# jhuldr/BrainFM

Hardware: AMD Instinct MI355X
Metric: voxels/sec whole-volume multi-task inference, 256^3 tiled (higher is better)
Workload: dtype f16x3-split (fp32-grade); 1 GPU; 256^3 volume, reference tiling win160/stride80 -> 27 tiles, UNet3D f64 x6 levels, 9 heads (69 ch), fused tail + deformed atlas + on-device stitch of 17 keys; stitched_keys=17, mfma_passes=3, submission=hipGraph replay per tile shape, parallelism=tiles sharded over 1 rank(s), gather to rank 0, tiles_in_flight_per_gpu=2

## Files before the change

### brainfm_amd/csrc/conv3d_wino4.hip

```cpp
#include "wino_shared.h"
#include <cstdlib>
#include <type_traits>

namespace {

typedef _Float16 half8 __attribute__((ext_vector_type(8)));
typedef float floatx16 __attribute__((ext_vector_type(16)));
typedef __fp16 fp16x2_t __attribute__((ext_vector_type(2)));

constexpr int KC = 16;
constexpr int NPOS = 6;
constexpr int NTHR = 256;
constexpr int NRG = NTHR / 32;
constexpr int MLD = 33;

struct W4Params {
    const float* A;
    int CA, D, H, W;
    const float *scale, *shift, *bound;
    int G;
    const uint4* wp;
    int wexp, Cout;
    float slope;
    float* out;
// ... 367 lines not shown
                float MN = INFINITY, MX = -INFINITY;
#pragma unroll
                for (int r = 0; r < NRG; ++r) {
                    Ssum += ls[r * 32 + tid]; Q += lq[r * 32 + tid];
                    MN = fminf(MN, lmn[r * 32 + tid]); MX = fmaxf(MX, lmx[r * 32 + tid]);
                }
                const size_t o = (size_t)mt * p.Cout + nt * 64 + nb * 32 + tid;
                p.rsum[o] = Ssum; p.rsq[o] = Q; p.rmn[o] = MN; p.rmx[o] = MX;
            }
        }
    }
}

template <int NPASS>
__global__ void __launch_bounds__(NTHR, 2) conv_wino4(const W4Params p) { conv_wino4_body<NPASS, 0>(p); }
template <int NPASS>
__global__ void __launch_bounds__(NTHR, 2) conv_wino4_masked(const W4Params p) { conv_wino4_body<NPASS, 1>(p); }

constexpr int DB_TD = 8, DB_TH = 8, DB_HT = 10, DB_NROW = 100;
constexpr int DB_PLANE = DB_NROW * 16;
constexpr int DB_RAWROW = 6 * 64;
constexpr int DB_RAW = DB_NROW * DB_RAWROW;
constexpr int DB_NDMA = DB_NROW / 2;
constexpr int DB_NDMA_WAVE = (DB_NDMA + 3) / 4;

template <bool LO>
__device__ __forceinline__ void split_store4_mix(const float (&t)[4], unsigned char* dp, int plane_stride) {
    const fp16x2_t h01 = __builtin_amdgcn_cvt_pkrtz(t[0], t[1]);
    const fp16x2_t h23 = __builtin_amdgcn_cvt_pkrtz(t[2], t[3]);
    uint2 hv;
    hv.x = __builtin_bit_cast(unsigned, h01);
    hv.y = __builtin_bit_cast(unsigned, h23);
    *reinterpret_cast<uint2*>(dp) = hv;
    if constexpr (LO) {
        uint2 lv;
        asm("v_fma_mixlo_f16 %0, %1, -1.0, %2 op_sel_hi:[1,0,0]" : "=v"(lv.x) : "v"(hv.x), "v"(t[0]));
        asm("v_fma_mixhi_f16 %0, %1, -1.0, %2 op_sel:[1,0,0] op_sel_hi:[1,0,0]" : "+v"(lv.x) : "v"(hv.x), "v"(t[1]));
        asm("v_fma_mixlo_f16 %0, %1, -1.0, %2 op_sel_hi:[1,0,0]" : "=v"(lv.y) : "v"(hv.y), "v"(t[2]));
        asm("v_fma_mixhi_f16 %0, %1, -1.0, %2 op_sel:[1,0,0] op_sel_hi:[1,0,0]" : "+v"(lv.y) : "v"(hv.y), "v"(t[3]));
        *reinterpret_cast<uint2*>(dp + plane_stride) = lv;
    }
}

template <int NPASS, int MODE, int ABL = 0>
__device__ __forceinline__ void conv_wino4d_body(const W4Params& pin) {
    W4Params p = pin;
    constexpr bool LIST = MODE != 0;
    constexpr bool UNI = MODE == 3;
    constexpr bool BY_FLAG = MODE == 2 || MODE == 3;
    constexpr int NPL = (NPASS == 3) ? 2 : 1;
    constexpr int NF = 2 * NPL;
    constexpr int NWF = 3 * NPL;
    constexpr int RAW_OFF = 2 * NPOS * NPL * DB_PLANE;
    extern __shared__ __attribute__((aligned(16))) unsigned char lds[];

    const int tid = threadIdx.x;
    const int lane = tid & 63;
    const int wv = __builtin_amdgcn_readfirstlane(tid >> 6);
    const int posA = wv;
    const int posB = 4 + (wv >> 1), nbB = wv & 1;
    const int l32 = lane & 31, khalf = lane >> 5;
#ifdef BFM_W4_ABLATE
    if (p.dbg_sleep > 0 && blockIdx.x < 512) {
        unsigned hwid;
        asm volatile("s_getreg_b32 %0, hwreg(HW_REG_HW_ID)" : "=s"(hwid));
        if (hwid & 1)
            for (int i = 0; i < p.dbg_sleep; ++i) __builtin_amdgcn_s_sleep(16);
    }
#endif
    int item;
    {
        const int nblk = LIST ? p.list_n[0] * p.NT : p.nMt * p.NT;
        const int bid = blockIdx.x;
        if (LIST && bid >= nblk) return;
        const int q = nblk >> 3, r = nblk & 7;
        const int xcd = bid & 7, idx = bid >> 3;
        item = (xcd < r ? xcd * (q + 1) : r * (q + 1) + (xcd - r) * q) + idx;
    }
    const int mt = LIST ? p.list[item / p.NT] : item / p.NT;
    const int nt = item % p.NT;
    int mtl = mt;
    if (!LIST && p.nMtS > 0) {
        const int smp = mt / p.nMtS;
        mtl = mt - smp * p.nMtS;
        p.A += smp * p.sA;
        p.out += smp * p.sO;
        p.scale += smp * p.saff;
        p.shift += smp * p.saff;
        p.bound += smp * p.G;
    }
    const int tx = mtl % p.nTx;
    const int ty = (mtl / p.nTx) % p.nTy;
    const int tz = mtl / (p.nTx * p.nTy);
    const int z0 = tz * DB_TD, y0 = ty * DB_TH, x0 = tx * 4;
    int cls = 0;
    if constexpr (BY_FLAG) cls = __builtin_amdgcn_readfirstlane((int)p.uni_flags[mt]);
    const bool rep = MODE == 2 && cls != 0;
    float4* const ybuf = BY_FLAG && cls ? reinterpret_cast<float4*>(p.uni_acc) + ((size_t)(cls - 1) * p.NT + nt) * (2 * 8 * NTHR) + tid
                                        : nullptr;

    float bmax = 0.f;
    for (int g = 0; g < p.G; ++g) bmax = fmaxf(bmax, p.bound[g]);
    int aexp = 0;
    if (bmax > 0.f && bmax < INFINITY) {
        int ex;
        (void)frexpf(bmax, &ex);
        aexp = 10 - ex;
        aexp = aexp > 60 ? 60 : (aexp < -60 ? -60 : aexp);
    }
    const float a_scale = ldexpf(1.0f, aexp);
    const float dq = ldexpf(1.0f, -(aexp + p.wexp));

    floatx16 acc[2][2];
    floatx16 accB[2];
    if constexpr (!UNI) {
    int a_off[4];
#pragma unroll
    for (int u = 0; u < 4; ++u) {
        const int pos = u < 2 ? posA : posB, mb = u & 1;
        const int pr = row_perm(l32);
        const int d = mb * 2 + (pr >> 4) + 4 * ((pr & 15) >> 3), h = pr & 7;
        a_off[u] = ((pos * 2 + khalf) * NPL) * DB_PLANE + (d * DB_HT + h) * 16;
    }

    const int q4 = tid & 3;
    int msk[2];
#pragma unroll
    for (int it = 0; it < 2; ++it) {
        const int r = (tid >> 2) + 64 * it;
        msk[it] = -1;
        if (r < DB_NROW) {
            const int hz = r / DB_HT, hy = r - hz * DB_HT;
            const int gz = z0 + hz - 1, gy = y0 + hy - 1;
            int m = 0;
            if (gz >= 0 && gz < p.D && gy >= 0 && gy < p.H) {
#pragma unroll
                for (int i = 0; i < 6; ++i)
                    if (x0 - 1 + i >= 0 && x0 - 1 + i < p.W) m |= 1 << i;
            }
            msk[it] = m;
        }
    }
    const bool inner = z0 >= 1 && z0 + DB_TD < p.D && y0 >= 1 && y0 + DB_TH < p.H && x0 >= 1 && x0 + 4 < p.W;
    const int st_plane = ((q4 >> 1) * NPL) * DB_PLANE + (q4 & 1) * 8;

    const int slot = lane >> 2;
    const int sb = slot >= 6 ? 1 : 0;
    int gxc = x0 + (slot - 6 * sb) - 1;
    gxc = gxc < 0 ? 0 : (gxc > p.W - 1 ? p.W - 1 : gxc);
    const int lane_el = gxc * p.CA + (lane & 3) * 4;
    const bool dma_lane = slot < 12;
    const unsigned raw_lds = (unsigned)(__UINTPTR_TYPE__)((__attribute__((address_space(3))) unsigned char*)(lds + RAW_OFF));
    const int zs = z0 > 0 ? z0 - 1 : 0;
    const float* slab = p.A + (int64_t)zs * p.H * p.W * p.CA;
    auto issue_dma = [&](int kc) __attribute__((always_inline)) {
        if constexpr ((ABL & 8) != 0) return;
        if (dma_lane) {
            int wvo = wv;
            asm volatile("" : "+s"(wvo));
#pragma unroll
            for (int n = 0; n < DB_NDMA_WAVE; ++n) {
                const int i = wvo + 4 * n;
                if (n < DB_NDMA_WAVE - 1 || i < DB_NDMA) {
                    const int hz = i / 5, hp = i - 5 * hz;
                    int gz = z0 + hz - 1;
                    gz = gz < 0 ? 0 : (gz > p.D - 1 ? p.D - 1 : gz);
                    int gy0 = y0 + 2 * hp - 1, gy1 = gy0 + 1;
                    gy0 = gy0 < 0 ? 0 : (gy0 > p.H - 1 ? p.H - 1 : gy0);
                    gy1 = gy1 > p.H - 1 ? p.H - 1 : gy1;
                    const unsigned ro0 = (unsigned)((((gz - zs) * p.H + gy0) * p.W) * p.CA);
                    const unsigned ro1 = (unsigned)((((gz - zs) * p.H + gy1) * p.W) * p.CA);
                    const unsigned vo = ((sb ? ro1 : ro0) + (unsigned)lane_el) * 4u;
                    const unsigned la = raw_lds + (unsigned)(i * (2 * DB_RAWROW));
                    asm volatile("s_mov_b32 m0, %2\n\ts_nop 0\n\tglobal_load_lds_dwordx4 %0, %1" ::"v"(vo), "s"(slab + kc * KC), "s"(la)
                                 : "memory");
                }
            }
        }
    };

#pragma unroll
    for (int u = 0; u < 2; ++u) {
#pragma unroll
        for (int i = 0; i < 16; ++i) { acc[u][0][i] = 0.f; acc[u][1][i] = 0.f; accB[u][i] = 0.f; }
    }

// ... 11 lines not shown
    };
    issue_dma(0);
    fetch(0, wq[0]);
    fetch(1, wq[1]);
    half8 a_abl[4][NPL];
    if constexpr ((ABL & 2) != 0) {
#pragma unroll
        for (int u = 0; u < 4; ++u)
#pragma unroll
            for (int hl = 0; hl < NPL; ++hl)
#pragma unroll
                for (int j = 0; j < 8; ++j) a_abl[u][hl][j] = (_Float16)(0.01f * (float)((lane * 7 + u * 3 + hl * 5 + j) % 61) - 0.3f);
    }

    for (int kc = 0; kc < p.KCN; ++kc) {
        const int c0 = kc * KC;
        const float4 sc4 = *reinterpret_cast<const float4*>(p.scale + c0 + q4 * 4);
        const float4 sh4 = *reinterpret_cast<const float4*>(p.shift + c0 + q4 * 4);
        const float sc[4] = {sc4.x * a_scale, sc4.y * a_scale, sc4.z * a_scale, sc4.w * a_scale};
        const float sh[4] = {sh4.x * a_scale, sh4.y * a_scale, sh4.z * a_scale, sh4.w * a_scale};
        __builtin_amdgcn_s_waitcnt(0x0F70);
        __syncthreads();
#pragma unroll
        for (int it = 0; it < 2; ++it) {
            if (msk[it] < 0) continue;
            if constexpr ((ABL & 4) != 0) continue;
            const int r = (tid >> 2) + 64 * it;
            const float4* rp = reinterpret_cast<const float4*>(
                __builtin_assume_aligned(lds + RAW_OFF + r * DB_RAWROW + q4 * 16, 16));
            float4 v[6];
#pragma unroll
            for (int i = 0; i < 6; ++i) v[i] = rp[i * 4];
            float dd[6][4];
            if (inner) {
#pragma unroll
                for (int i = 0; i < 6; ++i) {
                    const float y[4] = {v[i].x, v[i].y, v[i].z, v[i].w};
#pragma unroll
                    for (int c = 0; c < 4; ++c) dd[i][c] = fmaf(y[c], sc[c], sh[c]);
                }
            } else {
#pragma unroll
                for (int i = 0; i < 6; ++i) {
                    const bool ok = msk[it] & (1 << i);
                    const float y[4] = {v[i].x, v[i].y, v[i].z, v[i].w};
#pragma unroll
                    for (int c = 0; c < 4; ++c) {
                        const float a = fmaf(y[c], sc[c], sh[c]);
                        dd[i][c] = ok ? a : 0.f;
                    }
// ... 63 lines not shown
                    const half8 bhi = __builtin_bit_cast(half8, wq[cur][NF]);
                    if constexpr (NPASS == 3) {
                        const half8 blo = __builtin_bit_cast(half8, wq[cur][NF + 1]);
                        accB[u - 2] = __builtin_amdgcn_mfma_f32_32x32x16_f16(a[1], bhi, accB[u - 2], 0, 0, 0);
                        accB[u - 2] = __builtin_amdgcn_mfma_f32_32x32x16_f16(a[0], blo, accB[u - 2], 0, 0, 0);
                    }
                    accB[u - 2] = __builtin_amdgcn_mfma_f32_32x32x16_f16(a[0], bhi, accB[u - 2], 0, 0, 0);
                }
            }
        }
    }

    }

    if constexpr ((ABL & 16) != 0) {
        float sm = 0.f;
#pragma unroll
        for (int u = 0; u < 2; ++u)
#pragma unroll
            for (int i = 0; i < 16; ++i) sm += acc[u][0][i] + acc[u][1][i] + accB[u][i];
        if (sm == 12345.678f) p.out[tid] = sm;
        return;
    }
    float* m = reinterpret_cast<float*>(lds);
    const int col = tid & 31, rg = tid >> 5;
    const bool interior = z0 + DB_TD <= p.D && y0 + DB_TH <= p.H && x0 + 4 <= p.W;
    int un[4];
#pragma unroll
    for (int c = 0; c < 4; ++c) un[c] = row_unperm(16 * (c >> 1) + 8 * (c & 1) + rg);
    const unsigned off_t = (unsigned)((rg * p.W) * p.Cout + col);
#pragma unroll
    for (int nb = 0; nb < 2; ++nb) {
        if constexpr (!UNI && (ABL & 256) == 0) {
        __syncthreads();
#pragma unroll
        for (int u = 0; u < 2; ++u) {
            float* mw = m + (posA * 64 + u * 32 + khalf * 4) * MLD + l32;
#pragma unroll
            for (int i = 0; i < 16; ++i)
                mw[((i >> 2) * 8 + (i & 3)) * MLD] = acc[u][nb][i];
        }
        if (nbB == nb) {
#pragma unroll
            for (int u = 0; u < 2; ++u) {
                float* mw = m + (posB * 64 + u * 32 + khalf * 4) * MLD + l32;
#pragma unroll
                for (int i = 0; i < 16; ++i)
                    mw[((i >> 2) * 8 + (i & 3)) * MLD] = accB[u][i];
// ... 65 lines not shown
                    const float* mr = mc + qr * MLD;
                    const float m0 = mr[0 * 64 * MLD], m1 = mr[1 * 64 * MLD], m2 = mr[2 * 64 * MLD];
                    const float m3 = mr[3 * 64 * MLD], m4 = mr[4 * 64 * MLD], m5 = mr[5 * 64 * MLD];
                    const float s1 = m1 + m2, d1 = m1 - m2, s2 = m3 + m4, d2 = m3 - m4;
                    y[0] = ((m0 + s1) + s2) * dq;
                    y[1] = fmaf(2.f, d2, d1) * dq;
                    y[2] = fmaf(4.f, s2, s1) * dq;
                    y[3] = (fmaf(8.f, d2, d1) + m5) * dq;
                    if (MODE == 2 && rep) ybuf[(nb * 8 + it) * NTHR] = make_float4(y[0], y[1], y[2], y[3]);
                }
#pragma unroll
                for (int k = 0; k < 4; ++k) {
                    if (x0 + k < p.W) {
                        float r = y[k];
                        if (p.accum) r = r + o[off_t + (unsigned)(k * p.Cout)];
                        r = r >= 0.f ? r : r * p.slope;
                        o[off_t + (unsigned)(k * p.Cout)] = r;
                        fs += r; fq = fmaf(r, r, fq); fmn = fminf(fmn, r); fmx = fmaxf(fmx, r);
                    }
                }
            }
        }
        if (p.rsum != nullptr) {
            double* ls = reinterpret_cast<double*>(lds + (UNI ? (size_t)0 : (size_t)NPOS * 64 * MLD * sizeof(float)));
            double* lq = ls + NRG * 32;
            float* lmn = reinterpret_cast<float*>(lq + NRG * 32);
            float* lmx = lmn + NRG * 32;
            ls[rg * 32 + col] = (double)fs; lq[rg * 32 + col] = (double)fq;
            lmn[rg * 32 + col] = fmn; lmx[rg * 32 + col] = fmx;
            __syncthreads();
            if (tid < 32) {
                double Ssum = 0.0, Q = 0.0;
                float MN = INFINITY, MX = -INFINITY;
#pragma unroll
                for (int r = 0; r < NRG; ++r) {
                    Ssum += ls[r * 32 + tid]; Q += lq[r * 32 + tid];
                    MN = fminf(MN, lmn[r * 32 + tid]); MX = fmaxf(MX, lmx[r * 32 + tid]);
                }
                const size_t o = (size_t)mt * p.Cout + nt * 64 + nb * 32 + tid;
                p.rsum[o] = Ssum; p.rsq[o] = Q; p.rmn[o] = MN; p.rmx[o] = MX;
            }
        }
    }
}

template <int NPASS>
__global__ void __launch_bounds__(NTHR, 2) conv_wino4d(const W4Params p) { conv_wino4d_body<NPASS, 0>(p); }
template <int NPASS>
__global__ void __launch_bounds__(NTHR, 2) conv_wino4d_masked(const W4Params p) { conv_wino4d_body<NPASS, 1>(p); }
template <int NPASS>
__global__ void __launch_bounds__(NTHR, 2) conv_wino4d_rest(const W4Params p) { conv_wino4d_body<NPASS, 2>(p); }
template <int NPASS>
__global__ void __launch_bounds__(NTHR, 2) conv_wino4d_uniform(const W4Params p) { conv_wino4d_body<NPASS, 3>(p); }
#ifdef BFM_W4_ABLATE
template <int ABL>
__global__ void __launch_bounds__(NTHR, 2) conv_wino4d_abl(const W4Params p) { conv_wino4d_body<3, 0, ABL>(p); }
#endif

__global__ void pack_wino4(const float* __restrict__ w, int Cin, int Cout, int wexp, int npl, uint4* __restrict__ out) {
    const int KCN = Cin / KC;
    const int nf = 2 * npl;
    const int64_t n = (int64_t)(Cout / 64) * NPOS * KCN * 9 * nf * 64;
    const double s = ldexp(1.0, wexp);
    for (int64_t i = (int64_t)blockIdx.x * blockDim.x + threadIdx.x; i < n; i += (int64_t)gridDim.x * blockDim.x) {
        const int lane = (int)(i & 63);
        int64_t r = i >> 6;
        const int f = (int)(r % nf); r /= nf;
        const int t = (int)(r % 9); r /= 9;
        const int kc = (int)(r % KCN); r /= KCN;
        const int ps = (int)(r % NPOS); r /= NPOS;
        const int ntile = (int)r;
        const int nb = f / npl, hl = f - nb * npl;
        const int co = ntile * 64 + nb * 32 + (lane & 31);
        const int ci0 = kc * KC + 8 * (lane >> 5);
        half8 v;
#pragma unroll
// ... 12 lines not shown
        }
        out[i] = __builtin_bit_cast(uint4, v);
    }
}

int ilog2i(int v) { int r = 0; while ((1 << r) < v) ++r; return r; }

bool choose_box4(int D, int H, int W, int npl, int& TD, int& TH, int& TW) {
    if (!bfm_wino_choose_box(D, H, W, npl, TD, TH, TW)) return false;
    if (TW % 4 || TD * TH * (TW / 4) != 64) return false;
    const int64_t npos = (int64_t)(TD + 2) * (TH + 2) * (TW / 4);
    if (npos * 4 > 3 * NTHR) return false;
    const int64_t plane = ((npos * 16 + 255) / 256) * 256 + 16;
    return 2 * NPOS * npl * plane <= 62 * 1024;
}

bool use_dma_kernel(int D, int H, int W) {
#ifdef BFM_W4_ABLATE
    if (getenv("BFM_W4_OLD")) return false;
#endif
    return D >= DB_TD && H >= DB_TH && W >= 4;
}

bool choose_box_any(int D, int H, int W, int npl, int& TD, int& TH, int& TW) {
    if (use_dma_kernel(D, H, W)) { TD = DB_TD; TH = DB_TH; TW = 4; return true; }
    return choose_box4(D, H, W, npl, TD, TH, TW);
}

}

extern "C" size_t bfm_pack_conv_weights_wino4_bytes(int Cin, int Cout, int passes) {
    if (Cin <= 0 || Cout <= 0 || Cin % KC || Cout % 64) return 0;
    const int npl = passes == 3 ? 2 : 1;
    return (size_t)(Cout / 64) * NPOS * (Cin / KC) * 9 * 2 * npl * 64 * sizeof(uint4);
}

extern "C" int bfm_pack_conv_weights_wino4(const float* w_oidhw, int Cin, int Cout, float wmax_abs_host, int passes,
                                           void* wpacked, int* wexp_host, bfm_stream_t stream) {
    if (!w_oidhw || !wpacked || !wexp_host || Cin <= 0 || Cout <= 0) return BFM_E_ARG;
    if (Cin % KC || Cout % 64 || (passes != 1 && passes != 3)) return BFM_E_SHAPE;
    int wexp = 0;
    if (wmax_abs_host > 0.f && wmax_abs_host < INFINITY) {
        int ex;
        (void)frexpf(wmax_abs_host, &ex);
        wexp = 14 - ex;
        wexp = wexp > 60 ? 60 : (wexp < -60 ? -60 : wexp);
// ... 7 lines not shown
    return bfm_launch_status();
}

extern "C" int bfm_conv3x3x3_wino4_rows(int D, int H, int W, int passes) {
    int TD, TH, TW;
    if (D <= 0 || H <= 0 || W <= 0 || !choose_box_any(D, H, W, passes == 3 ? 2 : 1, TD, TH, TW)) return 0;
    return (int)bfm_box_count(D, H, W, TD, TH, TW);
}

extern "C" int bfm_conv3x3x3_wino4_box(int D, int H, int W, int passes, int* box) {
    int TD, TH, TW;
    if (!box || D <= 0 || H <= 0 || W <= 0 || !choose_box_any(D, H, W, passes == 3 ? 2 : 1, TD, TH, TW)) return BFM_E_ARG;
    box[0] = TD; box[1] = TH; box[2] = TW;
    return BFM_OK;
}

extern "C" size_t bfm_conv3x3x3_wino4_masked_workspace(int D, int H, int W, int passes) {
    const int n = bfm_conv3x3x3_wino4_rows(D, H, W, passes);
    if (n <= 0) return 0;
    return MaskListBuf::bytes((size_t)n);
}

static int w4_launch(const WinoLaunch& a) {
    if (const int rc = bfm_wino_check(a, KC)) return rc;
    const int D = a.D, H = a.H, W = a.W, CA = a.CA, Cout = a.Cout, passes = a.passes;
    const int S = a.batch.S, affine_stride = a.batch.affine_stride;
    const int npl = passes == 3 ? 2 : 1;
    W4Params p{};
    p.A = a.A; p.CA = CA; p.D = D; p.H = H; p.W = W;
    p.scale = a.scale; p.shift = a.shift; p.bound = a.bound; p.G = a.G;
    p.wp = static_cast<const uint4*>(a.wpacked);
    p.wexp = a.wexp; p.Cout = Cout; p.slope = a.slope; p.out = a.out; p.accum = a.flags & 1;
    if (!choose_box_any(D, H, W, npl, p.TD, p.TH, p.TW)) return BFM_E_SHAPE;
    const bool dma = use_dma_kernel(D, H, W);
    if (dma && (int64_t)(DB_TD + 2) * H * W * CA >= (int64_t)1 << 30) return BFM_E_SHAPE;
    p.HT = p.TH + 2; p.QW = p.TW / 4;
    p.qw_shift = ilog2i(p.QW); p.thq_shift = ilog2i(p.TH * p.QW);
    const int nTz = bfm_cdiv(D, p.TD);
    p.nTy = bfm_cdiv(H, p.TH); p.nTx = bfm_cdiv(W, p.TW);
    p.nMt = nTz * p.nTy * p.nTx;
    if (S > 1 || affine_stride > 0) {
        if (a.mask.img || S < 1 || (affine_stride != 0 && (affine_stride < CA || (affine_stride & 3)))) return BFM_E_ARG;
        p.nMtS = p.nMt;
        p.nMt = S * p.nMtS;
        p.saff = affine_stride > 0 ? affine_stride : CA;
        p.sA = (int64_t)D * H * W * CA;
        p.sO = (int64_t)D * H * W * Cout;
    }
    p.NT = Cout / 64;
    p.KCN = CA / KC;
    p.npos_lds = (p.TD + 2) * p.HT * p.QW;
    p.plane_stride = ((p.npos_lds * 16 + 255) / 256) * 256 + 16;
    size_t smem = dma ? (size_t)2 * NPOS * npl * DB_PLANE + DB_RAW : (size_t)2 * NPOS * npl * p.plane_stride;
    const size_t epi = (size_t)NPOS * 64 * MLD * sizeof(float) + (size_t)NRG * 32 * 24;
    if (smem < epi) smem = epi;
    if (smem > (dma ? 80u : 64u) * 1024) return BFM_E_SHAPE;
    const UniformFlagBuf fb{a.uniform.flags, (size_t)p.nMt};
    if (fb.flags) {
        int bd, bh, bw;
        if (!dma || a.mask.img || S > 1 || affine_stride > 0 || !a.uniform.scratch) return BFM_E_ARG;
        if (!bfm_wino_choose_box(D, H, W, npl, bd, bh, bw) || bd != p.TD || bh != p.TH || bw != p.TW) return BFM_E_SHAPE;
        p.uni_flags = fb.flags;
        p.uni_acc = a.uniform.scratch;
    }
    if (dma) {
        static bool attr = false;
        if (const int rc = bfm_raise_lds_limit(
                attr,
                {bfm_kernel(&conv_wino4d_rest<3>), bfm_kernel(&conv_wino4d_rest<1>), bfm_kernel(&conv_wino4d<3>),
                 bfm_kernel(&conv_wino4d<1>), bfm_kernel(&conv_wino4d_masked<3>), bfm_kernel(&conv_wino4d_masked<1>)},
                80 * 1024))
            return rc;
    }
    MomentRows rows;
    if (a.moment_rows && !rows.carve(a.moment_rows, (size_t)p.nMt * Cout)) return BFM_E_ARG;
    rows.into(p);
    if ((int64_t)p.nMt * p.NT > 0x7fffffff) return BFM_E_SHAPE;
    const dim3 grid((unsigned)(p.nMt * p.NT)), block(NTHR);
    hipStream_t st = bfm_s(a.stream);
    if (a.mask.img) {
        if (!a.mask.ws) return BFM_E_ARG;
        const MaskListBuf mb{a.mask.ws, (size_t)p.nMt};
        if (const int rc = bfm_wino_mask_list(a.mask.img, D, H, W, p.TD, p.TH, p.TW, p.nTy, p.nTx, p.nMt, a.mask.ws, a.stream))
            return rc;
        p.list = mb.list(); p.list_n = mb.count();
        if (dma) bfm_launch_by_passes(passes, conv_wino4d_masked<3>, conv_wino4d_masked<1>, grid, block, smem, st, p);
        else bfm_launch_by_passes(passes, conv_wino4_masked<3>, conv_wino4_masked<1>, grid, block, smem, st, p);
        return bfm_launch_status();
    }
    if (fb.flags) {
        p.list = fb.rest_list(); p.list_n = fb.counts();
        bfm_launch_by_passes(passes, conv_wino4d_rest<3>, conv_wino4d_rest<1>, grid, block, smem, st, p);
        p.list = fb.uniform_list(); p.list_n = fb.counts() + 1;
        bfm_launch_by_passes(passes, conv_wino4d_uniform<3>, conv_wino4d_uniform<1>, grid, block, 6144, st, p);
        return bfm_launch_status();
    }
#ifdef BFM_W4_ABLATE
    if (const char* e = getenv("BFM_W4_SLEEP")) p.dbg_sleep = atoi(e);
    if (const char* e = getenv("BFM_W4_ABL")) {
        const int abl = atoi(e);
        if (dma) {
#define W4D_ATTR(N) (void)hipFuncSetAttribute(reinterpret_cast<const void*>(&conv_wino4d_abl<N>), hipFuncAttributeMaxDynamicSharedMemorySize, 80 * 1024)
            W4D_ATTR(0); W4D_ATTR(1); W4D_ATTR(2); W4D_ATTR(3); W4D_ATTR(4); W4D_ATTR(8); W4D_ATTR(12); W4D_ATTR(15); W4D_ATTR(16); W4D_ATTR(31); W4D_ATTR(64); W4D_ATTR(28); W4D_ATTR(128); W4D_ATTR(256); W4D_ATTR(384); W4D_ATTR(512);
            switch (abl) {
#define W4D_CASE(N) case N: hipLaunchKernelGGL(conv_wino4d_abl<N>, grid, dim3(NTHR), smem, st, p); return bfm_launch_status()
                W4D_CASE(0); W4D_CASE(1); W4D_CASE(2); W4D_CASE(3); W4D_CASE(4); W4D_CASE(8); W4D_CASE(12); W4D_CASE(15); W4D_CASE(16); W4D_CASE(31); W4D_CASE(64); W4D_CASE(28); W4D_CASE(128); W4D_CASE(256); W4D_CASE(384); W4D_CASE(512);
                default: return BFM_E_ARG;
            }
        }
    }
#endif
    if (dma) bfm_launch_by_passes(passes, conv_wino4d<3>, conv_wino4d<1>, grid, block, smem, st, p);
    else bfm_launch_by_passes(passes, conv_wino4<3>, conv_wino4<1>, grid, block, smem, st, p);
    return bfm_launch_status();
}

extern "C" int bfm_conv3x3x3_wino4(const float* A, int CA, int D, int H, int W, const float* scale, const float* shift,
                                   const float* bound, int G, const void* wpacked, int wexp, int Cout, float slope,
                                   int passes, int flags, float* out, void* moment_rows, bfm_stream_t stream) {
    return w4_launch({A, CA, D, H, W, scale, shift, bound, G, wpacked, wexp, Cout, slope, passes, flags, out, moment_rows, stream});
}

extern "C" int bfm_conv3x3x3_wino4_batch(const float* A, int CA, int S, int D, int H, int W, const float* scale,
                                         const float* shift, const float* bound, int G, const void* wpacked, int wexp,
                                         int Cout, float slope, int passes, int flags, float* out, void* moment_rows,
                                         int affine_stride, bfm_stream_t stream) {
    if (S < 1) return BFM_E_ARG;
    WinoLaunch a{A, CA, D, H, W, scale, shift, bound, G, wpacked, wexp, Cout, slope, passes, flags, out, moment_rows, stream};
    a.batch = {S, affine_stride > 0 ? affine_stride : CA};
    return w4_launch(a);
}

extern "C" int bfm_conv3x3x3_wino4_masked(const float* A, int CA, int D, int H, int W, const float* scale, const float* shift,
                                          const float* bound, int G, const void* wpacked, int wexp, int Cout, float slope,
                                          int passes, int flags, float* out, const float* mask_image, void* workspace,
                                          size_t workspace_bytes, bfm_stream_t stream) {
    if (!mask_image || (flags & ~1)) return BFM_E_ARG;
    if (!workspace || (reinterpret_cast<uintptr_t>(workspace) & 3) ||
        workspace_bytes < bfm_conv3x3x3_wino4_masked_workspace(D, H, W, passes))
        return BFM_E_ARG;
    WinoLaunch a{A, CA, D, H, W, scale, shift, bound, G, wpacked, wexp, Cout, slope, passes, flags, out, nullptr, stream};
    a.mask = {mask_image, workspace};
    return w4_launch(a);
}

extern "C" size_t bfm_conv3x3x3_wino4_uniform_scratch(int Cout) {
    if (Cout <= 0 || Cout % 64) return 0;
    return (size_t)27 * (Cout / 64) * 2 * 8 * NTHR * sizeof(float4);
}

extern "C" int bfm_conv3x3x3_wino4_uniform(const float* A, int CA, int D, int H, int W, const float* scale, const float* shift,
                                           const float* bound, int G, const void* wpacked, int wexp, int Cout, float slope,
                                           int passes, int flags, float* out, void* moment_rows,
                                           const unsigned char* uniform_flags, void* scratch, bfm_stream_t stream) {
    if (!uniform_flags || !scratch || (reinterpret_cast<uintptr_t>(uniform_flags) & 3) || (reinterpret_cast<uintptr_t>(scratch) & 15))
        return BFM_E_ARG;
    WinoLaunch a{A, CA, D, H, W, scale, shift, bound, G, wpacked, wexp, Cout, slope, passes, flags, out, moment_rows, stream};
    a.uniform = {uniform_flags, static_cast<float*>(scratch)};
    return w4_launch(a);
}
// ... 1 lines not shown
```

### brainfm_amd/csrc/wino_shared.h

```cpp
#pragma once
#include "conv_shared.h"

bool bfm_wino_choose_box(int D, int H, int W, int npl, int& TD, int& TH, int& TW);

static inline size_t bfm_pad4(size_t n) { return (n + 3) & ~(size_t)3; }

struct MaskListBuf {
    void* ws;
    size_t n;
    static size_t bytes(size_t n) { return bfm_pad4(n) + 4 + n * 4; }
    unsigned char* act() const { return static_cast<unsigned char*>(ws); }
    int* count() const { return reinterpret_cast<int*>(act() + bfm_pad4(n)); }
    int* list() const { return count() + 1; }
};

struct UniformFlagBuf {
    const unsigned char* flags;
    size_t n;
    static size_t bytes(size_t n) { return bfm_pad4(n) + 27 * 4 + 2 * 4 + 2 * n * 4; }
    int* first() const { return reinterpret_cast<int*>(const_cast<unsigned char*>(flags) + bfm_pad4(n)); }
    int* counts() const { return first() + 27; }
    int* rest_list() const { return counts() + 2; }
    int* uniform_list() const { return rest_list() + n; }
};

int bfm_wino_mask_list(const float* mask_img, int D, int H, int W, int TD, int TH, int TW, int nTy, int nTx, int nMt, void* ws,
                       bfm_stream_t stream);

struct WinoLaunch {
    const float* A;
    int CA, D, H, W;
    const float *scale, *shift, *bound;
    int G;
    const void* wpacked;
    int wexp, Cout;
    float slope;
    int passes, flags;
    float* out;
    void* moment_rows;
    bfm_stream_t stream;
    struct { const float* img = nullptr; void* ws = nullptr; } mask;
    struct { const unsigned char* flags = nullptr; float* scratch = nullptr; } uniform;
    struct { float* out = nullptr; void* rows = nullptr; } pool;
    struct { int S = 1, affine_stride = 0; } batch;
};

static inline int bfm_wino_check(const WinoLaunch& a, int KC) {
    if (a.flags & ~1) return BFM_E_ARG;
    if (!a.A || a.CA <= 0 || a.D <= 0 || a.H <= 0 || a.W <= 0 || !a.scale || !a.shift || !a.bound || a.G <= 0 || !a.wpacked ||
        !a.out)
        return BFM_E_ARG;
    if (a.CA % KC || a.Cout % 64 || a.Cout <= 0) return BFM_E_SHAPE;
    if (a.passes != 1 && a.passes != 3) return BFM_E_ARG;
    if ((reinterpret_cast<uintptr_t>(a.A) & 15) || (reinterpret_cast<uintptr_t>(a.scale) & 15) ||
        (reinterpret_cast<uintptr_t>(a.shift) & 15) || (reinterpret_cast<uintptr_t>(a.wpacked) & 15) ||
        (reinterpret_cast<uintptr_t>(a.out) & 15))
        return BFM_E_ARG;
    if ((int64_t)a.D * a.H * a.W * a.CA > 0x7fffffffLL) return BFM_E_SHAPE;
    return BFM_OK;
}
```

### brainfm_amd/engine.py

```python
import ctypes as C
import os
from collections import OrderedDict, namedtuple

import numpy as np
import torch

from . import _lib as L

LABELS_LEFT = [0, 1, 2, 3, 4, 7, 8, 9, 10, 14, 15, 17, 31, 34, 36, 38, 40, 42]
LABELS_FULL = [0, 11, 12, 13, 16, 31, 32, 33, 34, 35, 36, 37, 38, 39, 40, 41, 42, 43, 44, 46,
               1, 2, 3, 4, 5, 6, 7, 8, 9, 10, 14, 15, 17, 47, 49, 51, 53, 55,
               18, 19, 20, 21, 22, 23, 24, 25, 26, 27, 28, 29, 30, 48, 50, 52, 54, 56]


def features_per_level(f_maps, num_levels):
    return [f_maps * 2 ** k for k in range(num_levels)]


def nearest_index_map(n_in, n_out):
    scale = np.float32(n_in) / np.float32(n_out)
    idx = np.floor(np.arange(n_out, dtype=np.float32) * scale).astype(np.int64)
    return np.minimum(idx, n_in - 1).astype(np.int32)


# ... 482 lines not shown
                                                     L.ptr(self._gn_ticket()) if self.gn_one_launch else None, st),
                    "gn_stats_rows " + ly.name)
            return ws
        wsb = self.lib.bfm_gn_stats_workspace(ca, cb, D, H, W, upp)
        ws = self._workspace(max(wsb, ws_min))
        L.check(self.lib.bfm_gn_stats_train(L.ptr(A), ca, L.ptr(B), cb, D, H, W, upp, L.ptr(ly.gamma), L.ptr(ly.beta),
                                            ly.groups, self.eps, L.ptr(scale), L.ptr(shift), L.ptr(bound), L.ptr(mean),
                                            L.ptr(rstd), L.ptr(ws), ws.numel(), st), "gn_stats " + ly.name)
        return ws

    def _record(self, ly, A, B, dims, lo_dims, scale, shift, bound, out):
        if self.tape is not None:
            mean, rstd = self._last_moments
            self.tape.append(dict(ly=ly, A=A, B=B, dims=tuple(dims), lo_dims=tuple(lo_dims) if lo_dims is not None else None,
                                  scale=scale, shift=shift, bound=bound, mean=mean, rstd=rstd, out=out))

    def _conv_launch(self, ly, A, ca, B, cb, dims, upp, scale, shift, bound, groups, cfg, out, ws, rows=None, slope=None,
                     mask_img=None, uni_flags=None, pool=None):
        D, H, W = dims
        st = L.stream_ptr()
        slope = self.slope if slope is None else float(slope)
        self._pack(ly, True, cfg[6])
        v = self._variant(cfg[6])
        if mask_img is not None:
            if v.masked is None or cb or rows is not None:
                raise L.BfmError("a masked launch is a one-source Winograd kernel without moment rows")
            nws = v.masked_workspace(D, H, W, self.passes)
            mws = torch.empty(nws, dtype=torch.uint8, device=self.device)
            L.check(v.masked(L.ptr(A), ca, D, H, W, L.ptr(scale), L.ptr(shift), L.ptr(bound), groups, L.ptr(ly.wpacked),
                             ly.wexp, ly.cout, slope, self.passes, cfg[7] & 1, L.ptr(out), L.ptr(mask_img), L.ptr(mws), nws,
                             st), "conv_wino(masked) " + ly.name)
            return
        if pool is not None:
            if cfg[6] != 3 or cb or mask_img is not None:
                raise L.BfmError("the fused pooling is the one-source F(2,3) kernel's")
            pooled, prow = pool
            if uni_flags is not None:
                scratch = torch.empty(self.lib.bfm_conv3x3x3_wino_uniform_scratch(ly.cout), dtype=torch.uint8,
                                      device=self.device)
                L.check(self.lib.bfm_conv3x3x3_wino_uniform_pool(
                    L.ptr(A), ca, D, H, W, L.ptr(scale), L.ptr(shift), L.ptr(bound), groups, L.ptr(ly.wpacked), ly.wexp,
                    ly.cout, slope, self.passes, cfg[7] & 1, L.ptr(out), L.ptr(rows[0]) if rows is not None else None,
                    L.ptr(uni_flags), L.ptr(scratch), L.ptr(pooled), L.ptr(prow[0]) if prow is not None else None, st),
                        "conv_wino(uniform, pool) " + ly.name)
            else:
                L.check(self.lib.bfm_conv3x3x3_wino_pool(
                    L.ptr(A), ca, D, H, W, L.ptr(scale), L.ptr(shift), L.ptr(bound), groups, L.ptr(ly.wpacked), ly.wexp,
                    ly.cout, slope, self.passes, cfg[7] & 1, L.ptr(out), L.ptr(rows[0]) if rows is not None else None,
                    L.ptr(pooled), L.ptr(prow[0]) if prow is not None else None, st), "conv_wino(pool) " + ly.name)
            return
        if uni_flags is not None and cfg[6] == 4 and not self._same_boxes(dims):
            uni_flags = None
        if uni_flags is not None and v.uniform is not None and not cb:
            scratch = torch.empty(v.uniform_scratch(ly.cout), dtype=torch.uint8, device=self.device)
            L.check(v.uniform(L.ptr(A), ca, D, H, W, L.ptr(scale), L.ptr(shift), L.ptr(bound), groups, L.ptr(ly.wpacked),
                              ly.wexp, ly.cout, slope, self.passes, cfg[7] & 1, L.ptr(out),
                              L.ptr(rows[0]) if rows is not None else None, L.ptr(uni_flags), L.ptr(scratch), st),
                    "conv_wino(uniform) " + ly.name)
            return
        if v.dense is not None:
            if cb:
                raise L.BfmError("the Winograd variant takes one source" if cfg[6] == 3 else
                                 "the Winograd variants take one source")
            L.check(v.dense(L.ptr(A), ca, D, H, W, L.ptr(scale), L.ptr(shift), L.ptr(bound), groups, L.ptr(ly.wpacked),
                            ly.wexp, ly.cout, slope, self.passes, cfg[7] & 1, L.ptr(out),
                            L.ptr(rows[0]) if rows is not None else None, st), "conv_%s %s" % (v.layout, ly.name))
            return
        L.check(self.lib.bfm_conv3x3x3_mfma_ex(L.ptr(A), ca, L.ptr(B) if cb else None, cb, D, H, W, upp if cb else None,
                                               L.ptr(scale), L.ptr(shift), L.ptr(bound), groups, L.ptr(ly.wpacked),
                                               ly.wexp, ly.cout, slope, self.passes, cfg, L.ptr(out), L.ptr(ws),
                                               ws.numel(), L.ptr(rows[0]) if rows is not None else None, st),
                "conv_mfma " + ly.name)

    def _needs_f23(self, ly):
        if self._f23_ids is None:
            self._f23_ids = {id(self.enc[i][j]) for i, j in ((0, 1), (1, 0), (1, 1)) if i < len(self.enc)}
        return id(ly) in self._f23_ids

    def _same_boxes(self, dims):
        if self._same_box_cache is None:
            self._same_box_cache = {}
        cache, key = self._same_box_cache, tuple(dims)
        if key not in cache:
            b3, b4 = (C.c_int * 3)(), (C.c_int * 3)()
            ok = (self._variant(3).box(dims[0], dims[1], dims[2], self.passes, b3) == 0 and
                  self._variant(4).box(dims[0], dims[1], dims[2], self.passes, b4) == 0)
            cache[key] = ok and list(b3) == list(b4)
        return cache[key]
# ... 260 lines not shown
        if self.tape is not None:
            self.tape.append(dict(pool_in=X, pool_dims=tuple(dims)))
        return out, (D // 2, H // 2, W // 2)

    def maxpool_batch(self, X, dims):
        S, (D, H, W), c = X.shape[0], dims, X.shape[-1]
        out = torch.empty((S, D // 2, H // 2, W // 2, c), dtype=torch.float32, device=self.device)
        if c % 4 or self.tape is not None:
            for s_ in range(S):
                self.maxpool(X[s_], dims, out=out[s_])
            return out
        rows = self._rows_buf(c, S, self.lib.bfm_maxpool2_batch_rows, c, D, H, W)
        L.check(self.lib.bfm_maxpool2_batch(L.ptr(X), c, S, D, H, W, L.ptr(out), L.ptr(rows[0]) if rows is not None else None,
                                            L.stream_ptr()), "maxpool2_batch")
        if rows is not None:
            out._bfm_rows = rows
        return out

    deep_from = int(os.environ.get("BFM_DEEP_FROM", "3"))
    deep_batch = os.environ.get("BFM_DEEP_BATCH", "1") != "0"
    DEEP_VERS = (0, 2)
    DEEP_VERS_1SRC = (0, 2, 4)
    use_wino_b5 = os.environ.get("BFM_WINO_B5", "1")
    deep_upfold = os.environ.get("BFM_DEEP_UPFOLD", "1") != "0"
    deep_upfold_min = int(os.environ.get("BFM_DEEP_UPFOLD_MIN", "100"))
    use_tap = os.environ.get("BFM_TAP", "1") != "0"
    tap_max = 64
    mask_skip = os.environ.get("BFM_MASK_SKIP", "1") != "0"
    uniform_skip = os.environ.get("BFM_UNIFORM_SKIP", "1") != "0"

    deep_vox = int(os.environ.get("BFM_DEEP_VOX", "16000"))

    def _region_ok(self, df):
        if self._deep_ok is None:
            self._deep_ok = {}
        cache = self._deep_ok
        if df not in cache:
            ndeep = len(self.enc) - 1 - df
            layers = [ly for pair in self.enc[df:] + self.dec[:ndeep] for ly in pair]
            cache[df] = all(ly.cin % 16 == 0 and ly.cout % 64 == 0 for ly in layers) and \
                self.enc[df - 1][1].cout % 16 == 0
        return cache[df]

    def has_deep_region(self):
        if not (self.deep_batch and self.tape is None and not self.force_direct and len(self.fm) > self.deep_from >= 1):
            return False
# ... 103 lines not shown
            return cfg
        if self.use_wino_b5 == "force" or os.environ.get("BFM_CONV_VER") == "5":
            cfg5[6] = 5
        elif key5 not in self._tuned:
            cfg5 = self._autotune(ly, key5, launch, vers=(cfg[6], 5))
        return cfg5

    def _batch_launch(self, ly, cfg, A, B, upp, dims, scale, shift, bound, out, rows=None, aff=0):
        S, (D, H, W), ca = A.shape[0], dims, A.shape[-1]
        cb = 0 if B is None else B.shape[-1]
        st = L.stream_ptr()
        self._pack(ly, True, cfg[6])
        if cfg[6] == 5:
            ws = self._workspace(self.lib.bfm_conv3x3x3_wino_b5_workspace(ca, ly.cout, S, D, H, W))
            L.check(self.lib.bfm_conv3x3x3_wino_b5_batch(L.ptr(A), ca, S, D, H, W, L.ptr(scale), L.ptr(shift), L.ptr(bound),
                                                         ly.groups, L.ptr(ly.wpacked), ly.wexp, ly.cout, self.slope,
                                                         self.passes, cfg[7] & 1, L.ptr(out),
                                                         L.ptr(rows[0]) if rows is not None else None, aff, L.ptr(ws),
                                                         ws.numel(), st), "conv_wino_b5_batch " + ly.name)
            return
        if cfg[6] == 4:
            L.check(self.lib.bfm_conv3x3x3_wino4_batch(L.ptr(A), ca, S, D, H, W, L.ptr(scale), L.ptr(shift), L.ptr(bound),
                                                       ly.groups, L.ptr(ly.wpacked), ly.wexp, ly.cout, self.slope, self.passes,
                                                       cfg[7] & 1, L.ptr(out), L.ptr(rows[0]) if rows is not None else None,
                                                       aff, st), "conv_wino4_batch " + ly.name)
            return
        ws = self._workspace(self.lib.bfm_conv3x3x3_mfma_batch_workspace(ly.cin, ly.cout, S, D, H, W, cfg[5]))
        L.check(self.lib.bfm_conv3x3x3_mfma_batch(L.ptr(A), ca, L.ptr(B) if cb else None, cb, S, D, H, W,
                                                  upp if cb else None, L.ptr(scale), L.ptr(shift), L.ptr(bound), ly.groups,
                                                  L.ptr(ly.wpacked), ly.wexp, ly.cout, self.slope, self.passes, cfg,
                                                  L.ptr(out), L.ptr(ws), ws.numel(),
                                                  L.ptr(rows[0]) if rows is not None else None, aff, st),
                "conv_mfma_batch " + ly.name)

    def _batch_conv_upfold(self, ly, A, dims, B, lo_dims, scale, shift, bound):
        S = A.shape[0]
        D, H, W = dims
        ca, cb = A.shape[-1], B.shape[-1]
        st = L.stream_ptr()
        sk = self._skip_layer(ly, ca)
        if "upfold" not in ly.packs:
            self._make_upfold_pack(ly, ca, cb)
        ly.touch("upfold")
        wup, wexp_up = ly.packs["upfold"]
        sc_a, sh_a = scale[:, :ca], shift[:, :ca]
        sc_b, sh_b = scale[:, ca:], shift[:, ca:]
        aff = ca + cb
        out = torch.empty((S, D, H, W, ly.cout), dtype=torch.float32, device=self.device)
# ... 434 lines not shown
```

Baseline: 218.3 million voxels/s.

## Add 512-thread wide Winograd-4 kernel sharing input tile across two output-channel tiles

Adds a wide variant of the DMA Winograd-4 conv kernel in which one 512-thread block computes two 64-channel output tiles over the same spatial box. The input slab is DMA-staged and split once and shared by both halves, which removes duplicate input loads and transforms and halves the grid size. Each half gets its own epilogue region in LDS. A heuristic enables it only when Cout is a multiple of 128, there is no mask, and the last wave of blocks is well filled; env flags can force or disable it. The cost is doubled epilogue LDS and larger blocks, which may lower occupancy.

```diff
diff --git a/brainfm_amd/csrc/conv3d_wino4.hip b/brainfm_amd/csrc/conv3d_wino4.hip
--- a/brainfm_amd/csrc/conv3d_wino4.hip
+++ b/brainfm_amd/csrc/conv3d_wino4.hip
@@ -413,7 +413,6 @@
 constexpr int DB_RAWROW = 6 * 64;
 constexpr int DB_RAW = DB_NROW * DB_RAWROW;
 constexpr int DB_NDMA = DB_NROW / 2;
-constexpr int DB_NDMA_WAVE = (DB_NDMA + 3) / 4;
 
 template <bool LO>
 __device__ __forceinline__ void split_store4_mix(const float (&t)[4], unsigned char* dp, int plane_stride) {
@@ -433,8 +432,10 @@
     }
 }
 
-template <int NPASS, int MODE, int ABL = 0>
+template <int NPASS, int MODE, int ABL = 0, int NW = 4>
 __device__ __forceinline__ void conv_wino4d_body(const W4Params& pin) {
+    static_assert(NW == 4 || (NW == 8 && (MODE == 0 || MODE == 2)), "the wide form: dense and rest only");
+    constexpr bool WIDE = NW == 8;
     W4Params p = pin;
     constexpr bool LIST = MODE != 0;
     constexpr bool UNI = MODE == 3;
@@ -447,7 +448,10 @@
 
     const int tid = threadIdx.x;
     const int lane = tid & 63;
-    const int wv = __builtin_amdgcn_readfirstlane(tid >> 6);
+    const int wv8 = __builtin_amdgcn_readfirstlane(tid >> 6);
+    const int wv = WIDE ? wv8 & 3 : wv8;
+    const int hf = WIDE ? wv8 >> 2 : 0;
+    const int ht = WIDE ? tid & (NTHR - 1) : tid;
     const int posA = wv;
     const int posB = 4 + (wv >> 1), nbB = wv & 1;
     const int l32 = lane & 31, khalf = lane >> 5;
@@ -459,17 +463,18 @@
             for (int i = 0; i < p.dbg_sleep; ++i) __builtin_amdgcn_s_sleep(16);
     }
 #endif
+    const int NTW = WIDE ? p.NT >> 1 : p.NT;
     int item;
     {
-        const int nblk = LIST ? p.list_n[0] * p.NT : p.nMt * p.NT;
+        const int nblk = LIST ? p.list_n[0] * NTW : p.nMt * NTW;
         const int bid = blockIdx.x;
         if (LIST && bid >= nblk) return;
         const int q = nblk >> 3, r = nblk & 7;
         const int xcd = bid & 7, idx = bid >> 3;
         item = (xcd < r ? xcd * (q + 1) : r * (q + 1) + (xcd - r) * q) + idx;
     }
-    const int mt = LIST ? p.list[item / p.NT] : item / p.NT;
-    const int nt = item % p.NT;
+    const int mt = LIST ? p.list[item / NTW] : item / NTW;
+    const int nt = WIDE ? 2 * (item % NTW) + hf : item % NTW;
     int mtl = mt;
     if (!LIST && p.nMtS > 0) {
         const int smp = mt / p.nMtS;
@@ -487,7 +492,7 @@
     int cls = 0;
     if constexpr (BY_FLAG) cls = __builtin_amdgcn_readfirstlane((int)p.uni_flags[mt]);
     const bool rep = MODE == 2 && cls != 0;
-    float4* const ybuf = BY_FLAG && cls ? reinterpret_cast<float4*>(p.uni_acc) + ((size_t)(cls - 1) * p.NT + nt) * (2 * 8 * NTHR) + tid
+    float4* const ybuf = BY_FLAG && cls ? reinterpret_cast<float4*>(p.uni_acc) + ((size_t)(cls - 1) * p.NT + nt) * (2 * 8 * NTHR) + ht
                                         : nullptr;
 
     float bmax = 0.f;
@@ -514,11 +519,12 @@
         a_off[u] = ((pos * 2 + khalf) * NPL) * DB_PLANE + (d * DB_HT + h) * 16;
     }
 
+    constexpr int NIT = WIDE ? 1 : 2, RSTEP = NW * 16;
     const int q4 = tid & 3;
-    int msk[2];
-#pragma unroll
-    for (int it = 0; it < 2; ++it) {
-        const int r = (tid >> 2) + 64 * it;
+    int msk[NIT];
+#pragma unroll
+    for (int it = 0; it < NIT; ++it) {
+        const int r = (tid >> 2) + RSTEP * it;
         msk[it] = -1;
         if (r < DB_NROW) {
             const int hz = r / DB_HT, hy = r - hz * DB_HT;
@@ -541,18 +547,19 @@
     gxc = gxc < 0 ? 0 : (gxc > p.W - 1 ? p.W - 1 : gxc);
     const int lane_el = gxc * p.CA + (lane & 3) * 4;
     const bool dma_lane = slot < 12;
+    constexpr int NDMA_WAVE = (DB_NDMA + NW - 1) / NW;
     const unsigned raw_lds = (unsigned)(__UINTPTR_TYPE__)((__attribute__((address_space(3))) unsigned char*)(lds + RAW_OFF));
     const int zs = z0 > 0 ? z0 - 1 : 0;
     const float* slab = p.A + (int64_t)zs * p.H * p.W * p.CA;
     auto issue_dma = [&](int kc) __attribute__((always_inline)) {
         if constexpr ((ABL & 8) != 0) return;
         if (dma_lane) {
-            int wvo = wv;
+            int wvo = wv8;
             asm volatile("" : "+s"(wvo));
 #pragma unroll
-            for (int n = 0; n < DB_NDMA_WAVE; ++n) {
-                const int i = wvo + 4 * n;
-                if (n < DB_NDMA_WAVE - 1 || i < DB_NDMA) {
+            for (int n = 0; n < NDMA_WAVE; ++n) {
+                const int i = wvo + NW * n;
+                if (n < NDMA_WAVE - 1 || i < DB_NDMA) {
                     const int hz = i / 5, hp = i - 5 * hz;
                     int gz = z0 + hz - 1;
                     gz = gz < 0 ? 0 : (gz > p.D - 1 ? p.D - 1 : gz);
@@ -610,10 +617,10 @@
         __builtin_amdgcn_s_waitcnt(0x0F70);
         __syncthreads();
 #pragma unroll
-        for (int it = 0; it < 2; ++it) {
+        for (int it = 0; it < NIT; ++it) {
             if (msk[it] < 0) continue;
             if constexpr ((ABL & 4) != 0) continue;
-            const int r = (tid >> 2) + 64 * it;
+            const int r = (tid >> 2) + RSTEP * it;
             const float4* rp = reinterpret_cast<const float4*>(
                 __builtin_assume_aligned(lds + RAW_OFF + r * DB_RAWROW + q4 * 16, 16));
             float4 v[6];
@@ -723,8 +730,10 @@
         if (sm == 12345.678f) p.out[tid] = sm;
         return;
     }
-    float* m = reinterpret_cast<float*>(lds);
-    const int col = tid & 31, rg = tid >> 5;
+    constexpr size_t EPI_HALF = (size_t)NPOS * 64 * MLD * sizeof(float) + (size_t)NRG * 32 * 24;
+    unsigned char* const lds_h = WIDE ? lds + hf * EPI_HALF : lds;
+    float* m = reinterpret_cast<float*>(lds_h);
+    const int col = ht & 31, rg = ht >> 5;
     const bool interior = z0 + DB_TD <= p.D && y0 + DB_TH <= p.H && x0 + 4 <= p.W;
     int un[4];
 #pragma unroll
@@ -836,22 +845,22 @@
             }
         }
         if (p.rsum != nullptr) {
-            double* ls = reinterpret_cast<double*>(lds + (UNI ? (size_t)0 : (size_t)NPOS * 64 * MLD * sizeof(float)));
+            double* ls = reinterpret_cast<double*>(lds_h + (UNI ? (size_t)0 : (size_t)NPOS * 64 * MLD * sizeof(float)));
             double* lq = ls + NRG * 32;
             float* lmn = reinterpret_cast<float*>(lq + NRG * 32);
             float* lmx = lmn + NRG * 32;
             ls[rg * 32 + col] = (double)fs; lq[rg * 32 + col] = (double)fq;
             lmn[rg * 32 + col] = fmn; lmx[rg * 32 + col] = fmx;
             __syncthreads();
-            if (tid < 32) {
+            if (ht < 32) {
                 double Ssum = 0.0, Q = 0.0;
                 float MN = INFINITY, MX = -INFINITY;
 #pragma unroll
                 for (int r = 0; r < NRG; ++r) {
-                    Ssum += ls[r * 32 + tid]; Q += lq[r * 32 + tid];
-                    MN = fminf(MN, lmn[r * 32 + tid]); MX = fmaxf(MX, lmx[r * 32 + tid]);
-                }
-                const size_t o = (size_t)mt * p.Cout + nt * 64 + nb * 32 + tid;
+                    Ssum += ls[r * 32 + ht]; Q += lq[r * 32 + ht];
+                    MN = fminf(MN, lmn[r * 32 + ht]); MX = fmaxf(MX, lmx[r * 32 + ht]);
+                }
+                const size_t o = (size_t)mt * p.Cout + nt * 64 + nb * 32 + ht;
                 p.rsum[o] = Ssum; p.rsq[o] = Q; p.rmn[o] = MN; p.rmx[o] = MX;
             }
         }
@@ -866,6 +875,10 @@
 __global__ void __launch_bounds__(NTHR, 2) conv_wino4d_rest(const W4Params p) { conv_wino4d_body<NPASS, 2>(p); }
 template <int NPASS>
 __global__ void __launch_bounds__(NTHR, 2) conv_wino4d_uniform(const W4Params p) { conv_wino4d_body<NPASS, 3>(p); }
+template <int NPASS>
+__global__ void __launch_bounds__(2 * NTHR, 2) conv_wino4d_wide(const W4Params p) { conv_wino4d_body<NPASS, 0, 0, 8>(p); }
+template <int NPASS>
+__global__ void __launch_bounds__(2 * NTHR, 2) conv_wino4d_rest_wide(const W4Params p) { conv_wino4d_body<NPASS, 2, 0, 8>(p); }
 #ifdef BFM_W4_ABLATE
 template <int ABL>
 __global__ void __launch_bounds__(NTHR, 2) conv_wino4d_abl(const W4Params p) { conv_wino4d_body<3, 0, ABL>(p); }
@@ -924,6 +937,20 @@
     return D >= DB_TD && H >= DB_TH && W >= 4;
 }
 
+constexpr int W4W_CUS = 256;
+constexpr int W4_FLAG_NARROW = 4;
+constexpr int W4_FLAG_WIDE = 8;
+bool w4_wide_can(int Cout, int D, int H, int W, bool masked) {
+    return use_dma_kernel(D, H, W) && Cout % 128 == 0 && !masked;
+}
+bool w4_wide(int CA, int Cout, int D, int H, int W, int S, bool masked, bool pair) {
+    (void)CA;
+    if (pair || !w4_wide_can(Cout, D, H, W, masked)) return false;
+    const int64_t boxes = (int64_t)(S > 1 ? S : 1) * bfm_box_count(D, H, W, DB_TD, DB_TH, 4);
+    const int64_t last = boxes * (Cout / 128) % W4W_CUS;
+    return last == 0 || last > W4W_CUS / 2;
+}
+
 bool choose_box_any(int D, int H, int W, int npl, int& TD, int& TH, int& TW) {
     if (use_dma_kernel(D, H, W)) { TD = DB_TD; TH = DB_TH; TW = 4; return true; }
     return choose_box4(D, H, W, npl, TD, TH, TW);
@@ -977,7 +1004,7 @@
 }
 
 static int w4_launch(const WinoLaunch& a) {
-    if (const int rc = bfm_wino_check(a, KC)) return rc;
+    if (const int rc = bfm_wino_check(a, KC, 1 | W4_FLAG_NARROW | W4_FLAG_WIDE)) return rc;
     const int D = a.D, H = a.H, W = a.W, CA = a.CA, Cout = a.Cout, passes = a.passes;
     const int S = a.batch.S, affine_stride = a.batch.affine_stride;
     const int npl = passes == 3 ? 2 : 1;
@@ -1010,6 +1037,10 @@
     const size_t epi = (size_t)NPOS * 64 * MLD * sizeof(float) + (size_t)NRG * 32 * 24;
     if (smem < epi) smem = epi;
     if (smem > (dma ? 80u : 64u) * 1024) return BFM_E_SHAPE;
+    const bool wide = !(a.flags & W4_FLAG_NARROW) &&
+                      ((a.flags & W4_FLAG_WIDE) ? w4_wide_can(Cout, D, H, W, a.mask.img != nullptr)
+                                                : w4_wide(CA, Cout, D, H, W, S, a.mask.img != nullptr, a.uniform.flags != nullptr));
+    const size_t smem_w = 2 * epi;
     const UniformFlagBuf fb{a.uniform.flags, (size_t)p.nMt};
     if (fb.flags) {
         int bd, bh, bw;
@@ -1027,11 +1058,21 @@
                 80 * 1024))
             return rc;
     }
+    if (wide) {
+        static bool attr_w = false;
+        if (const int rc = bfm_raise_lds_limit(
+                attr_w,
+                {bfm_kernel(&conv_wino4d_wide<3>), bfm_kernel(&conv_wino4d_wide<1>), bfm_kernel(&conv_wino4d_rest_wide<3>),
+                 bfm_kernel(&conv_wino4d_rest_wide<1>)},
+                (int)smem_w))
+            return rc;
+    }
     MomentRows rows;
     if (a.moment_rows && !rows.carve(a.moment_rows, (size_t)p.nMt * Cout)) return BFM_E_ARG;
     rows.into(p);
     if ((int64_t)p.nMt * p.NT > 0x7fffffff) return BFM_E_SHAPE;
     const dim3 grid((unsigned)(p.nMt * p.NT)), block(NTHR);
+    const dim3 grid_w((unsigned)(p.nMt * (p.NT / 2))), block_w(2 * NTHR);
     hipStream_t st = bfm_s(a.stream);
     if (a.mask.img) {
         if (!a.mask.ws) return BFM_E_ARG;
@@ -1045,7 +1086,8 @@
     }
     if (fb.flags) {
         p.list = fb.rest_list(); p.list_n = fb.counts();
-        bfm_launch_by_passes(passes, conv_wino4d_rest<3>, conv_wino4d_rest<1>, grid, block, smem, st, p);
+        if (wide) bfm_launch_by_passes(passes, conv_wino4d_rest_wide<3>, conv_wino4d_rest_wide<1>, grid_w, block_w, smem_w, st, p);
+        else bfm_launch_by_passes(passes, conv_wino4d_rest<3>, conv_wino4d_rest<1>, grid, block, smem, st, p);
         p.list = fb.uniform_list(); p.list_n = fb.counts() + 1;
         bfm_launch_by_passes(passes, conv_wino4d_uniform<3>, conv_wino4d_uniform<1>, grid, block, 6144, st, p);
         return bfm_launch_status();
@@ -1065,7 +1107,8 @@
         }
     }
 #endif
-    if (dma) bfm_launch_by_passes(passes, conv_wino4d<3>, conv_wino4d<1>, grid, block, smem, st, p);
+    if (wide) bfm_launch_by_passes(passes, conv_wino4d_wide<3>, conv_wino4d_wide<1>, grid_w, block_w, smem_w, st, p);
+    else if (dma) bfm_launch_by_passes(passes, conv_wino4d<3>, conv_wino4d<1>, grid, block, smem, st, p);
     else bfm_launch_by_passes(passes, conv_wino4<3>, conv_wino4<1>, grid, block, smem, st, p);
     return bfm_launch_status();
 }
@@ -1090,7 +1133,7 @@
                                           const float* bound, int G, const void* wpacked, int wexp, int Cout, float slope,
                                           int passes, int flags, float* out, const float* mask_image, void* workspace,
                                           size_t workspace_bytes, bfm_stream_t stream) {
-    if (!mask_image || (flags & ~1)) return BFM_E_ARG;
+    if (!mask_image || (flags & ~(1 | W4_FLAG_NARROW | W4_FLAG_WIDE))) return BFM_E_ARG;
     if (!workspace || (reinterpret_cast<uintptr_t>(workspace) & 3) ||
         workspace_bytes < bfm_conv3x3x3_wino4_masked_workspace(D, H, W, passes))
         return BFM_E_ARG;
diff --git a/brainfm_amd/csrc/wino_shared.h b/brainfm_amd/csrc/wino_shared.h
--- a/brainfm_amd/csrc/wino_shared.h
+++ b/brainfm_amd/csrc/wino_shared.h
@@ -45,8 +45,8 @@
     struct { int S = 1, affine_stride = 0; } batch;
 };
 
-static inline int bfm_wino_check(const WinoLaunch& a, int KC) {
-    if (a.flags & ~1) return BFM_E_ARG;
+static inline int bfm_wino_check(const WinoLaunch& a, int KC, int flag_mask = 1) {
+    if (a.flags & ~flag_mask) return BFM_E_ARG;
     if (!a.A || a.CA <= 0 || a.D <= 0 || a.H <= 0 || a.W <= 0 || !a.scale || !a.shift || !a.bound || a.G <= 0 || !a.wpacked ||
         !a.out)
         return BFM_E_ARG;
diff --git a/brainfm_amd/engine.py b/brainfm_amd/engine.py
--- a/brainfm_amd/engine.py
+++ b/brainfm_amd/engine.py
@@ -528,13 +528,14 @@
         slope = self.slope if slope is None else float(slope)
         self._pack(ly, True, cfg[6])
         v = self._variant(cfg[6])
+        fl = (cfg[7] & 1) | (self._w4_flags() if cfg[6] == 4 else 0)
         if mask_img is not None:
             if v.masked is None or cb or rows is not None:
                 raise L.BfmError("a masked launch is a one-source Winograd kernel without moment rows")
             nws = v.masked_workspace(D, H, W, self.passes)
             mws = torch.empty(nws, dtype=torch.uint8, device=self.device)
             L.check(v.masked(L.ptr(A), ca, D, H, W, L.ptr(scale), L.ptr(shift), L.ptr(bound), groups, L.ptr(ly.wpacked),
-                             ly.wexp, ly.cout, slope, self.passes, cfg[7] & 1, L.ptr(out), L.ptr(mask_img), L.ptr(mws), nws,
+                             ly.wexp, ly.cout, slope, self.passes, fl, L.ptr(out), L.ptr(mask_img), L.ptr(mws), nws,
                              st), "conv_wino(masked) " + ly.name)
             return
         if pool is not None:
@@ -560,7 +561,7 @@
         if uni_flags is not None and v.uniform is not None and not cb:
             scratch = torch.empty(v.uniform_scratch(ly.cout), dtype=torch.uint8, device=self.device)
             L.check(v.uniform(L.ptr(A), ca, D, H, W, L.ptr(scale), L.ptr(shift), L.ptr(bound), groups, L.ptr(ly.wpacked),
-                              ly.wexp, ly.cout, slope, self.passes, cfg[7] & 1, L.ptr(out),
+                              ly.wexp, ly.cout, slope, self.passes, fl, L.ptr(out),
                               L.ptr(rows[0]) if rows is not None else None, L.ptr(uni_flags), L.ptr(scratch), st),
                     "conv_wino(uniform) " + ly.name)
             return
@@ -569,7 +570,7 @@
                 raise L.BfmError("the Winograd variant takes one source" if cfg[6] == 3 else
                                  "the Winograd variants take one source")
             L.check(v.dense(L.ptr(A), ca, D, H, W, L.ptr(scale), L.ptr(shift), L.ptr(bound), groups, L.ptr(ly.wpacked),
-                            ly.wexp, ly.cout, slope, self.passes, cfg[7] & 1, L.ptr(out),
+                            ly.wexp, ly.cout, slope, self.passes, fl, L.ptr(out),
                             L.ptr(rows[0]) if rows is not None else None, st), "conv_%s %s" % (v.layout, ly.name))
             return
         L.check(self.lib.bfm_conv3x3x3_mfma_ex(L.ptr(A), ca, L.ptr(B) if cb else None, cb, D, H, W, upp if cb else None,
@@ -876,6 +877,10 @@
     DEEP_VERS = (0, 2)
     DEEP_VERS_1SRC = (0, 2, 4)
     use_wino_b5 = os.environ.get("BFM_WINO_B5", "1")
+    use_w4_wide = os.environ.get("BFM_W4_WIDE", "1")
+
+    def _w4_flags(self):
+        return {"0": 4, "force": 8}.get(self.use_w4_wide, 0)
     deep_upfold = os.environ.get("BFM_DEEP_UPFOLD", "1") != "0"
     deep_upfold_min = int(os.environ.get("BFM_DEEP_UPFOLD_MIN", "100"))
     use_tap = os.environ.get("BFM_TAP", "1") != "0"
@@ -1025,8 +1030,9 @@
         if cfg[6] == 4:
             L.check(self.lib.bfm_conv3x3x3_wino4_batch(L.ptr(A), ca, S, D, H, W, L.ptr(scale), L.ptr(shift), L.ptr(bound),
                                                        ly.groups, L.ptr(ly.wpacked), ly.wexp, ly.cout, self.slope, self.passes,
-                                                       cfg[7] & 1, L.ptr(out), L.ptr(rows[0]) if rows is not None else None,
-                                                       aff, st), "conv_wino4_batch " + ly.name)
+                                                       (cfg[7] & 1) | self._w4_flags(), L.ptr(out),
+                                                       L.ptr(rows[0]) if rows is not None else None, aff, st),
+                    "conv_wino4_batch " + ly.name)
             return
         ws = self._workspace(self.lib.bfm_conv3x3x3_mfma_batch_workspace(ly.cin, ly.cout, S, D, H, W, cfg[5]))
         L.check(self.lib.bfm_conv3x3x3_mfma_batch(L.ptr(A), ca, L.ptr(B) if cb else None, cb, S, D, H, W,
```

Result: no change. 218.7 million voxels/s, median of 2 (+0.2%).
